# MPEGGroup/mpeg-pcc-tmc13

Hardware: AMD Instinct MI355X
Metric: RAHT forward+inverse attribute-transform Mpoints/s (bit-exact vs CPU reference) (higher is better)
Workload: dtype int64 (Q15 fixed point), int32 I/O

## Files before the change

### mpeg-pcc-tmc13_amd/csrc/cx_level.hpp

```cpp
#pragma once

#include "cx_tree.hpp"
#include "raht_arith.hpp"
#include "raht_levels.hpp"
#include "raht_links.hpp"
#include "raht_rdoq.hpp"

#ifndef GPCC_CX_SEARCH_ARY
#define GPCC_CX_SEARCH_ARY 2
#endif
#ifndef GPCC_CX_SEARCH_MASKED
#define GPCC_CX_SEARCH_MASKED 0
#endif

namespace gpcc {

constexpr int kCxG = 57;
constexpr int kCxSlices = 64;
constexpr int kCxTopTiles = 8;

struct CxCtx {
  TreeView tv;
  CxLists cl;
  const gpcc_raht_params* params;
// ... 128 lines not shown
{
  if (w <= 65536)
    return (int64_t)(1 + (((w << 30) * (rs40 >> 15)) >> 40));
  return (int64_t)isqrt(w << (2 * kFpFrac), L.rsqrt);
}

__device__ __forceinline__ CxNorm
cx_norm(int32_t w, const SharedLut& L)
{
  CxNorm r;
  if (w < kSmallN) {
    r.sq = L.norm_sq[w];
    r.rs = L.norm_rs[w];
    r.shift = 0;
    return r;
  }
  const uint64_t rs40 = irsqrt((uint64_t)w, L.rsqrt);
  r.shift = w > 1024 ? ilog2_u64((uint64_t)w - 1) >> 1 : 0;
  r.rs = (int64_t)(rs40 >> (40 - r.shift - kFpFrac));
  r.sq = cx_sqrt_from_rsqrt((uint64_t)w, rs40, L);
  return r;
}

template<class A>
__device__ __forceinline__ typename A::T
cx_scale(typename A::T v, const CxNorm& nm, typename A::Coef rs)
{
  return A::mulc(A::shr(v, nm.shift), rs);
}

template<class VT>
__device__ __forceinline__ VT
cx_bperm_v(int src_lane, VT v)
{
  return __builtin_bit_cast(VT, cx_bperm_i64(src_lane, __builtin_bit_cast(int64_t, v)));
}

__device__ __forceinline__ void
cx_coeffs(
  int32_t wl, int32_t wr, int64_t sql, int64_t sqr, const SharedLut& L, int64_t* a, int64_t* b,
  int64_t* sqw)
{
  const uint64_t w = (uint64_t)wl + (uint64_t)wr;
  if (wl < kSmallW && wr < kSmallW) {
    *a = L.bfly_a[wl * kSmallW + wr];
    *b = L.bfly_b[wl * kSmallW + wr];
    *sqw = L.norm_sq[w];
    return;
  }
  const uint64_t rs = irsqrt(w, L.rsqrt);
  *a = (int64_t)(((uint64_t)sql * rs) >> 40);
  *b = (int64_t)(((uint64_t)sqr * rs) >> 40);
  *sqw = cx_sqrt_from_rsqrt(w, rs, L);
}

__device__ __forceinline__ uint32_t
cx_rdoq_threshold(int64_t dist2, int64_t lambda, double inv_lambda, int rate_coeff, uint32_t limit)
{
  const uint64_t d = (uint64_t)dist2 << 26;
  const uint64_t lam = (uint64_t)lambda;
  const int rc = (rate_coeff + 128) >> 8;
  constexpr uint64_t kCap = 128;
  uint64_t q = kCap;
  if (d < lam * kCap) {
    q = (uint64_t)((double)d * inv_lambda);
    q -= q * lam > d;
    q += (q + 1) * lam <= d;
  }
  const int m = (int)q - rc + 1;
  if (m <= 1)
    return 0;
  if (m <= 2)
    return 1;
  if (m <= 3)
    return 2;
  if (m <= 5)
    return 3;
  if (m <= 7)
    return 5;
  if (m <= 9)
    return 7;
  if (m <= 11)
    return 9;
  int bb = (m - 12 + 1) >> 1;
  bb = bb < 1 ? 1 : bb;
  if (bb > 30)
    return kDescNever;
  const uint32_t tz = 10u + (1u << (bb - 1));
  return tz > limit ? kDescNever : tz;
}

__device__ __forceinline__ void
cx_fill_quant(ParamsConst prm, const LevelSched& e, int c, CxQuant* qt, int entry)
{
  int a0 = 0, a1 = 0;
  const int pos = entry - 1;
  if (pos >= 1 && e.ac_layer < prm->num_ac_qp_layers) {
    a0 = prm->ac_qp_offset[e.ac_layer][pos - 1][0];
    a1 = prm->ac_qp_offset[e.ac_layer][pos - 1][1];
  }
  Quantizer q[2];
  qpset_quantizers(prm, e.qp_layer, a0, a1, q);
  qt->q[entry][0] = q[0];
  qt->q[entry][1] = q[1];
  if (entry == 0) {
    const int64_t l0 = q[0].step;
    qt->lambda = l0 * l0 * (c == 1 ? 25 : 35);
    qt->inv_lambda = 1.0 / (double)qt->lambda;
  }
}

#ifdef GPCC_CX_PROF
__device__ unsigned long long g_cx_prof[16];
__device__ unsigned long long g_cx_prof_n[4];
struct CxProf {
  unsigned long long last;
  __device__ CxProf() { last = __builtin_amdgcn_s_memtime(); }
  __device__ void mark(int phase)
  {
    const unsigned long long t = __builtin_amdgcn_s_memtime();
    if (lane_id() == 0)
      atomicAdd(&g_cx_prof[phase], t - last);
    last = t;
  }
  __device__ void count(int slot, unsigned n)
  {
    if (lane_id() == 0)
      atomicAdd(&g_cx_prof[slot], (unsigned long long)n);
  }
};
#else
struct CxProf {
  __device__ void mark(int) {}
  __device__ void count(int, unsigned) {}
};
#endif

template<int C>
__device__ __forceinline__ void
cx_level_setup(const CxCtx& cx, CxSmem& sm, int li)
{
  const ParamsConst prm = (ParamsConst)cx.params;
// ... 427 lines not shown
  Quantizer qa[2], qr[2];
  int64_t lambda;
  double inv_lambda;
  if (S <= kCxSlices) {
    const CxQuant& qt = sm.qt[s];
    qa[0] = qt.q[1 + pos][0];
    qa[1] = qt.q[1 + pos][1];
    qr[0] = qt.q[0][0];
    qr[1] = qt.q[0][1];
    lambda = qt.lambda;
    inv_lambda = qt.inv_lambda;
  } else {
    int ac0 = 0, ac1 = 0;
    if (e.ac_layer < prm->num_ac_qp_layers && pos) {
      ac0 = prm->ac_qp_offset[e.ac_layer][pos - 1][0];
      ac1 = prm->ac_qp_offset[e.ac_layer][pos - 1][1];
    }
    qpset_quantizers(prm, e.qp_layer, ac0, ac1, qa);
    qpset_quantizers(prm, e.qp_layer, 0, 0, qr);
    const int64_t l0 = qr[0].step;
    lambda = l0 * l0 * (C == 1 ? 25 : 35);
    inv_lambda = 1.0 / (double)lambda;
  }

  const typename A::Quant qaa[2] = {A::quant(qa[0]), A::quant(qa[1])};
  int32_t qco[C];
#pragma unroll
  for (int k = 0; k < C; k++)
    qco[k] = 0;
  if (ENC) {
    uint32_t d = kDescZero;
    if (coded) {
      if (enable_pred) {
#pragma unroll
        for (int k = 0; k < C; k++)
          src[k] -= pred[k];
      }
      const typename A::Quant qra[2] = {A::quant(qr[0]), A::quant(qr[1])};
      int64_t sum_coeff = 0, dist2 = 0;
      int rate_coeff = 0;
#pragma unroll
      for (int k = 0; k < C; k++) {
        const VT co = A::round_int(src[k]);
        const int64_t coi = A::to_small(co);
        dist2 += coi * coi;
        int64_t aq = A::quantize(qra[k ? 1 : 0], co);
        aq = aq < 0 ? -aq : aq;
        sum_coeff += aq;
        rate_coeff += rate_log_small(aq);
        qco[k] = A::quantize(qaa[k ? 1 : 0], co);
      }
      d = kDescNever;
      if (sum_coeff < 3) {
        d = cx_rdoq_threshold(dist2, lambda, inv_lambda, rate_coeff, (uint32_t)sl.n_s);
        if (sum_coeff == 0)
          d |= kDescZero;
      }
    }

    prof.mark(4);
    const unsigned long long ep = (unsigned long long)(li + 1) << 48;
    unsigned long long todo = __ballot(coded);
    bool zero_me = false;
    bool published = false;
    while (todo) {
      const int first = __ffsll((long long)todo) - 1;
      const int s_cur = __shfl(s, first);
      const int c_first = __shfl(cblock, first);
      const bool mine = coded && s == s_cur;
      const unsigned long long seg = __ballot(mine);
      todo &= ~seg;
      const bool last_seg = todo == 0;
      const int ncoef = __popcll(seg);
      const int e_base = __shfl(e.coeff_base, first);
      const int e_par = __shfl((int)e.parity, first);
      const int c_end = __shfl(sl.coeff_end, first);
      if (mine)
        wdesc[cidx - c_first] = d;
      __builtin_amdgcn_wave_barrier();
      const bool valid = lane < ncoef;
      const uint32_t dd = valid ? wdesc[lane] : kDescZero;
      const int ci = c_first + lane;
      const bool starts = c_first == e_base;
      const bool ends = c_first + ncoef == c_end;
      int l_in = 0, l_out = 0;
      int tz;
      if (starts) {
        l_in = cx.slice_l[(e_par ^ 1) * S + s_cur];
        l_out = rdoq_chunk(dd, ci, valid, l_in, c_first, &tz);
        if (last_seg && lane == 0)
          __hip_atomic_store(
            &cx.tstate[tile], ep | (3ull << 32) | (uint32_t)l_out, __ATOMIC_RELAXED, __HIP_MEMORY_SCOPE_AGENT);
        published = published || last_seg;
      } else {
        const int la0 = -1, lb0 = c_first - 1;
        int tza, tzb;
        const int la = rdoq_chunk(dd, ci, valid, la0, c_first, &tza);
        const int lb = rdoq_chunk(dd, ci, valid, lb0, c_first, &tzb);
        const int status = lb == lb0 ? kTileTransparent : (la == lb ? kTileClosed : kTileOpen);
        if (last_seg && status != kTileOpen) {
          if (lane == 0)
            __hip_atomic_store(
              &cx.tstate[tile],
              ep | ((unsigned long long)(status == kTileClosed ? 2 : 1) << 32)
                | (uint32_t)(status == kTileClosed ? la : ncoef),
              __ATOMIC_RELAXED, __HIP_MEMORY_SCOPE_AGENT);
          published = true;
// ... 192 lines not shown
```

### mpeg-pcc-tmc13_amd/csrc/raht_levels.hpp

```cpp
#pragma once

#include "raht_common.hpp"

namespace gpcc {

enum LevelMode { kAnalyze = 0, kSynth = 1, kFused = 2, kLossySub = 3 };

constexpr uint32_t kDescNever = 0x7fffffffu;
constexpr uint32_t kDescZero = 0x80000000u;

typedef const __attribute__((address_space(4))) gpcc_raht_params* ParamsConst;

struct InterRef {
  const int64_t* pos;
  const int32_t* prefix;
  int32_t n_ref;
  int32_t lr;
  int32_t blocks;
  int32_t dual;
  int32_t filtered;
  const int32_t* tap;
  const int64_t* hkey;
  const int32_t* hfp;
  const int32_t* hlf;
// ... 155 lines not shown
  const int qp0 = clip(p->layer_qp[layer][0] + off0, 4, p->max_qp);
  const int qp1 = clip(p->layer_qp[layer][1] + off1 + qp0, 4, p->max_qp);
  q[0] = make_quantizer(qp0 + p->fixed_point_qp_offset);
  q[1] = make_quantizer(qp1 + p->fixed_point_qp_offset);
}

__device__ __forceinline__ int
find_in_window(
  const int64_t* __restrict__ key, int first, int last, int from,
  int64_t value, int64_t d)
{
  int lo, end;
  if (d >= 0) {
    lo = from;
    end = (d + 1 < (int64_t)(last - from)) ? from + (int)(d + 1) : last;
  } else {
    end = from;
    lo = (-d < (int64_t)(from - first)) ? from - (int)(-d) : first;
  }
  int hi = end;
  while (lo < hi) {
    const int mid = lo + ((hi - lo) >> 1);
    if (key[mid] < value)
      lo = mid + 1;
    else
      hi = mid;
  }
  if (lo == end)
    return -1;
  return key[lo] == value ? lo : -1;
}

__device__ __forceinline__ uint32_t
neigh_mask(int i)
{
  constexpr uint8_t m[19] = {255, 240, 204, 170, 192, 160, 136, 3,  5, 15,
                             17,  51,  85,  10,  34,  12,  68,  48, 80};
  return m[i];
}
__device__ __forceinline__ uint32_t
neigh_offset(int i)
{
  constexpr uint8_t o[19] = {0, 35, 21, 14, 49, 42, 28, 1,  2, 3,
                             4, 5,  6,  10, 12, 17, 20, 33, 34};
  return o[i];
}

__device__ __forceinline__ int
rate_log_small(int64_t aq)
{
  return aq == 0 ? 0 : (aq == 1 ? 256 : 406);
}

__device__ __forceinline__ uint32_t
rdoq_threshold(int64_t dist2, int64_t lambda, int rate_coeff, uint32_t limit)
{
  const uint64_t d = (uint64_t)dist2 << 26;
  const uint64_t lam = (uint64_t)lambda;
  const int rc = (rate_coeff + 128) >> 8;
  constexpr uint64_t kCap = 128;
  uint64_t q = kCap;
  if (d < lam * kCap) {
    q = (uint64_t)((double)d / (double)lam);
    q -= q * lam > d;
    q += (q + 1) * lam <= d;
  }
  const int m = (int)q - rc + 1;
  if (m <= 1)
    return 0;
  if (m <= 2)
    return 1;
  if (m <= 3)
    return 2;
  if (m <= 5)
    return 3;
  if (m <= 7)
    return 5;
  if (m <= 9)
    return 7;
  if (m <= 11)
    return 9;
  int bb = (m - 12 + 1) >> 1;
  bb = bb < 1 ? 1 : bb;
  if (bb > 30)
    return kDescNever;
  const uint32_t tz = 10u + (1u << (bb - 1));
  return tz > limit ? kDescNever : tz;
}

template<int C>
__global__ __launch_bounds__(256) void
raht_level_prepass_kernel(LevelCtx ctx)
{
  __shared__ int wave_cnt[4];
  __shared__ int base_s;
  if (tree_failed(ctx.tv))
    return;
  const TreeView& tv = ctx.tv;
  const int li = ctx.li;
  const bool ext = ctx.params->raht_extension != 0;
  const int num_parents = tv.soff[li + 1][tv.num_slices];
  const int lane = lane_id(), wave = threadIdx.x >> 6;
  if (ctx.rdoq_state && ctx.slice_l && blockIdx.x == 0)
    for (int s = threadIdx.x; s < tv.num_slices; s += blockDim.x)
      ctx.slice_l[(li & 1) * tv.num_slices + s] = ctx.slice_l[((li + 1) & 1) * tv.num_slices + s];
  const int64_t chunks = ((int64_t)num_parents + 255) >> 8;
  const int64_t per = (chunks + gridDim.x - 1) / gridDim.x;
  const int64_t gbeg = min((int64_t)blockIdx.x * per, chunks);
  const int64_t gend = min(gbeg + per, chunks);

  int mine = 0;
  for (int64_t chunk = gbeg; chunk < gend; chunk++) {
    const int j = (int)(chunk * 256) + threadIdx.x;
    if (j < num_parents) {
      const int s = find_slice(tv.soff[li + 1], tv.num_slices, j);
      if (ctx.sched[s].lvl[li].processed) {
        const int nchild = tv.fc[li + 1][j + 1] - tv.fc[li + 1][j];
        mine += !(ext && nchild == 1);
      }
    }
  }
#pragma unroll
  for (int d = 1; d < kWave; d <<= 1)
    mine += __shfl_xor(mine, d);
  if (lane == 0)
    wave_cnt[wave] = mine;
  __syncthreads();
  if (threadIdx.x == 0) {
    const unsigned long long ep = (unsigned long long)(li + 1) << 48;
    const unsigned total = wave_cnt[0] + wave_cnt[1] + wave_cnt[2] + wave_cnt[3];
    unsigned excl = 0;
    if (blockIdx.x > 0) {
      __hip_atomic_store(
        &ctx.scan_state[blockIdx.x], ep | (1ull << 32) | total, __ATOMIC_RELAXED,
        __HIP_MEMORY_SCOPE_AGENT);
      int k = (int)blockIdx.x - 1;
      for (;;) {
        const unsigned long long v = __hip_atomic_load(
          &ctx.scan_state[k], __ATOMIC_RELAXED, __HIP_MEMORY_SCOPE_AGENT);
        if ((v >> 48) != (unsigned long long)(li + 1)) {
// ... 70 lines not shown
```

### mpeg-pcc-tmc13_amd/csrc/raht_subnode.hpp

```cpp
#pragma once

#include <stdlib.h>

#include "raht_arith.hpp"
#include "raht_inter.hpp"
#include "raht_levels.hpp"
#include "raht_links.hpp"

namespace gpcc {

#ifndef GPCC_SUB_CHUNK
#define GPCC_SUB_CHUNK 1
#endif
#ifndef GPCC_SUB_DSTORE
#define GPCC_SUB_DSTORE 0
#endif
#ifndef GPCC_SUB_POLL_N
#define GPCC_SUB_POLL_N 1
#endif
#ifndef GPCC_SUB_IDLE_FAST
#define GPCC_SUB_IDLE_FAST 1
#endif
#ifndef GPCC_SUB_IDLE_SPIN
#define GPCC_SUB_IDLE_SPIN 0
#endif
__device__ __forceinline__ int64_t
sub_round_of_ticket(int tk, int cls)
{
  constexpr int K = GPCC_SUB_CHUNK;
  return ((int64_t)(tk / K) * 8 + cls) * K + tk % K;
}

#ifdef GPCC_SUB_PROF
__device__ unsigned long long g_sub_prof[16 + 32 * 20];
struct SubProf {
  unsigned long long t0 = 0, t1 = 0, last = 0, acc[4] = {0, 0, 0, 0}, iters = 0, idle_iters = 0;
  unsigned long long last2 = 0, sub_acc[6] = {0, 0, 0, 0, 0, 0}, execs[2] = {0, 0};
  template<int WHICH> __device__ void enter() { execs[WHICH]++; last2 = now(); }
  template<int K> __device__ void sub() { const unsigned long long t = now(); sub_acc[K] += t - last2; last2 = t; }
  __device__ static unsigned long long now() { return __builtin_amdgcn_s_memtime(); }
  __device__ void round_begin() { t0 = now(); }
  __device__ void loop_begin() { t1 = now(); }
  __device__ void iter_begin() { last = now(); iters++; }
  template<int STAGE> __device__ void mark() { const unsigned long long t = now(); acc[STAGE] += t - last; last = t; }
  __device__ void idle() { idle_iters++; }
  __device__ void round_end(int lane, int li)
  {
    if (lane != 0)
      return;
    const unsigned long long t2 = now();
    const unsigned long long v[9] = {1, t1 - t0, t2 - t1, acc[0], acc[1], acc[2], acc[3], iters, idle_iters};
    for (int i = 0; i < 9; i++)
      atomicAdd(&g_sub_prof[i], v[i]);
    atomicAdd(&g_sub_prof[16 + li * 4 + 0], 1ull);
    atomicAdd(&g_sub_prof[16 + li * 4 + 1], t1 - t0);
    atomicAdd(&g_sub_prof[16 + li * 4 + 2], t2 - t1);
    atomicAdd(&g_sub_prof[16 + li * 4 + 3], iters);
    for (int i = 0; i < 4; i++)
      atomicAdd(&g_sub_prof[144 + li * 6 + i], acc[i]);
    atomicAdd(&g_sub_prof[144 + li * 6 + 4], idle_iters);
    atomicAdd(&g_sub_prof[336 + li * 10 + 0], execs[0]);
    atomicAdd(&g_sub_prof[336 + li * 10 + 1], execs[1]);
    for (int i = 0; i < 6; i++)
      atomicAdd(&g_sub_prof[336 + li * 10 + 2 + i], sub_acc[i]);
  }
};
#else
struct SubProf {
  __device__ void round_begin() {}
  __device__ void loop_begin() {}
  __device__ void iter_begin() {}
  template<int STAGE> __device__ void mark() {}
  template<int WHICH> __device__ void enter() {}
  template<int K> __device__ void sub() {}
  __device__ void idle() {}
  __device__ void round_end(int, int) {}
};
// ... 4 lines not shown
{
#if GPCC_EXPERIMENTS
  auto rounds = [] {
    const char* e = getenv("GPCC_SUB_CLAIM");
    const int v = e ? atoi(e) : 1;
    return v < 1 ? 1 : (v > 64 ? 64 : v);
  };
  auto limit = [] {
    const char* e = getenv("GPCC_SUB_CLAIM_PARENTS");
    return e ? (int64_t)atoll(e) : (int64_t)100000;
  };
#ifdef GPCC_EMU
  const int r = rounds();
  const int64_t lim = limit();
#else
  static const int r = rounds();
  static const int64_t lim = limit();
#endif
  return (encoder && !haar && r > 1 && parents <= lim) ? r : 1;
#else
  (void)encoder;
  (void)haar;
  (void)parents;
  return 1;
#endif
}

__device__ __forceinline__ int
occu_shift(int i12)
{
  constexpr uint8_t s[12] = {6, 5, 4, 3, 2, 1, 3, 1, 2, 1, 2, 3};
  return s[i12];
}

__device__ __forceinline__ int32_t
load_agent_i32(const int32_t* p)
{
  return __hip_atomic_load(p, __ATOMIC_RELAXED, __HIP_MEMORY_SCOPE_AGENT);
}
__device__ __forceinline__ int64_t
load_agent_i64(const int64_t* p)
{
  return __hip_atomic_load(p, __ATOMIC_RELAXED, __HIP_MEMORY_SCOPE_AGENT);
}
__device__ __forceinline__ void
store_agent_i64(int64_t* p, int64_t v)
{
  __hip_atomic_store(p, v, __ATOMIC_RELAXED, __HIP_MEMORY_SCOPE_AGENT);
}

#ifndef GPCC_SUB_SLEEP
#define GPCC_SUB_SLEEP 4
#endif
#ifndef GPCC_SUB_POLL_RR
#define GPCC_SUB_POLL_RR 0
#endif
#ifndef GPCC_SUB_LOSSY_WAVES
#define GPCC_SUB_LOSSY_WAVES 3
#endif
#ifndef GPCC_SUB_SYNTH3_WAVES
#define GPCC_SUB_SYNTH3_WAVES 4
#endif
template<int C, int MODE, class A = ArithI64, bool INTER = false, bool REC = false>
__global__ __launch_bounds__(256, MODE == kLossySub ? GPCC_SUB_LOSSY_WAVES : (C == 3 ? GPCC_SUB_SYNTH3_WAVES : 4)) void
raht_level_sub_kernel(LevelCtx ctx)
{
  static_assert(!(REC && (INTER || MODE == kFused)), "records: fixed-point intra kernels only");
  static_assert(MODE == kSynth || MODE == kFused || MODE == kLossySub, "mode");
  static_assert(!(A::kF64 && MODE == kFused), "integer Haar is integer arithmetic");
  typedef typename A::T VT;
  typedef typename A::Coef VC;
  constexpr bool kLossy = MODE == kLossySub;
  __shared__ SharedLut lut_s;
  if (tree_failed(ctx.tv))
    return;
  load_lut(&lut_s, ctx.lut);
  const SharedLut& lut = lut_s;

  constexpr bool kEnc = MODE != kSynth;
  constexpr bool kRecon = true;
  const TreeView& tv = ctx.tv;
  const ParamsConst prm = (ParamsConst)ctx.params;
  const int li = ctx.li;
  const int t = threadIdx.x & 7;
  const int lane = lane_id();
  const int gbase = threadIdx.x & 56;
  const bool haar = !A::kF64 && prm->integer_haar_enable_flag != 0;
  const bool ext = A::kF64 || prm->raht_extension != 0;
  const int32_t epoch = li + 1;
#ifdef GPCC_EMU
  __shared__ unsigned long long wmail_s[8 * 4 * 64 * C];
  unsigned long long* wm = wmail_s + ((blockIdx.x & 7) * 4 + (threadIdx.x >> 6)) * (64 * C);
#else
  __shared__ unsigned long long wmail_s[4 * 64 * C];
  unsigned long long* wm = wmail_s + (threadIdx.x >> 6) * (64 * C);
#endif
  int pwc12[12];
#pragma unroll
  for (int i12 = 0; i12 < 12; i12++)
    pwc12[i12] = prm->pred_weight_child[i12];
  bool in_range = true;
  const int cls = blockIdx.x & 7;

  const int num_work = ctx.work_count[li];
#if GPCC_EXPERIMENTS
  const int claim_rounds = ctx.claim_rounds > 1 ? ctx.claim_rounds : 1;
  bool stop_all = false;
  for (;;) {
    int tk = 0;
    if (lane == 0)
      tk = atomicAdd(&ctx.ticket[li * 8 + (claim_rounds > 1 ? 0 : cls)], 1);
    tk = __shfl(tk, 0);
    const int64_t wround0 = claim_rounds > 1 ? (int64_t)tk * claim_rounds : sub_round_of_ticket(tk, cls);
    if (wround0 * 8 >= num_work || stop_all)
      break;
    bool carry_known = false;
    int carry_l = -1;
   for (int sr = 0; sr < claim_rounds; sr++) {
    const int64_t wround = wround0 + sr;
    if (wround * 8 >= num_work)
      break;
    SubProf prof;
    prof.round_begin();
    if (__hip_atomic_load(ctx.error, __ATOMIC_RELAXED, __HIP_MEMORY_SCOPE_AGENT)) {
      stop_all = true;
      break;
    }
#else
  for (;;) {
    int tk = 0;
    if (lane == 0)
      tk = atomicAdd(&ctx.ticket[li * 8 + cls], 1);
    tk = __shfl(tk, 0);
    const int64_t wround = sub_round_of_ticket(tk, cls);
    if (wround * 8 >= num_work)
      break;
    SubProf prof;
    prof.round_begin();
    if (__hip_atomic_load(ctx.error, __ATOMIC_RELAXED, __HIP_MEMORY_SCOPE_AGENT))
      break;
#endif
    const int wi = (int)(wround * 8) + (lane >> 3);
    const bool live = wi < num_work;
    const int j = live ? ctx.worklist[wi] : 0;
    int s = 0;
    LevelSched e;
    e.processed = 0;
    const size_t rln = REC ? (size_t)ctx.brec.lanes : 0;
    const size_t rat = (size_t)wround * 64 + lane;
    const int32_t* __restrict__ rf = REC ? ctx.brec.f32 + rat : nullptr;
    if (live) {
      if constexpr (REC)
        s = rf[kSfSlice * rln];
// ... 313 lines not shown
    const VC nrm_sq = A::coef(nrm_sq_i), nrm_rs = A::coef(nrm_rs_i);
    const typename A::Quant qaa[2] = {A::quant(qa[0]), A::quant(qa[1])};
    if (kEnc && !REC) {
      if (!haar && w > 1) {
#pragma unroll
        for (int k = 0; k < C; k++)
          src[k] = A::mulc(A::shr(src[k], nrm_shift), nrm_rs);
      }
#pragma unroll
      for (int k = 0; k < C; k++)
        in_range = in_range && A::below(src[k], A::kFwdLimit);
#pragma unroll
      for (int st = 0; st < 3; st++) {
        const int bit = 1 << st;
        const bool left = !(t & bit);
        const bool both = wl[st] && wr[st];
        const bool swap = !wl[st] && wr[st];
#pragma unroll
        for (int k = 0; k < C; k++) {
          const VT own = src[k], oth = shfl_xor_v(own, bit);
          if (both) {
            if (haar) {
              if constexpr (!A::kF64) {
                const int64_t hf = left ? oth - own : own - oth;
                src[k] = left ? own + ((hf >> (1 + kFpFrac)) << kFpFrac) : hf;
              }
            } else {
              src[k] = left ? A::mulc(oth, cb[st]) + A::mulc(own, ca[st])
                            : A::mulc(own, ca[st]) - A::mulc(oth, cb[st]);
            }
          } else if (swap) {
            src[k] = oth;
          }
        }
      }
    }
    const uint32_t coded_mask = group8_bits(coded);
    const int ncoef = popc32(coded_mask);
    const int crank = inherit_dc ? rank - 1 : rank;
    const int cfirst = e.coeff_base + (inherit_dc ? (c0 - sc0) - pj : 0);
    int rank_src = 0;
    if (kLossy) {
#pragma unroll
      for (int u = 0; u < 8; u++) {
        const int ru = __shfl(crank, gbase | u);
        if (((coded_mask >> u) & 1) && ru == t)
          rank_src = u;
      }
    }
    Quantizer qr[2] = {{1, 1}, {1, 1}};
    if (kLossy && coded)
      qpset_quantizers(prm, e.qp_layer, nq0, nq1, qr);
    const typename A::Quant qra[2] = {A::quant(qr[0]), A::quant(qr[1])};
    bool lin_known = false;
    int lin = -1;
    VT dc[C];
#pragma unroll
    for (int k = 0; k < C; k++)
      dc[k] = A::zero();
    if (on && inherit_dc && t == 0) {
#pragma unroll
      for (int k = 0; k < C; k++) {
        const int64_t val = par2(ctx.rec_us, par_par)[prow * C + k];
        dc[k] = A::from_i64(
          ext ? val : (val > 0 ? val << (kFpFrac - 2) : -((-val) << (kFpFrac - 2))));
        in_range = in_range && A::below(dc[k], A::kInvLimit);
      }
    }

    const bool run = do_search && enable_pred;
    const int64_t* __restrict__ prec = par2(ctx.rec, par_par);
    const int64_t rbase = (int64_t)pt0 - sp0;
    int wsum = 0;
    VT lim_lo = A::zero(), lim_hi = A::zero();
#pragma unroll
    for (int i = 0; i < 7; i++) {
      int q;
      if (i == 0)
        q = j;
      else
        q = __shfl(pn[0], gbase | (i - 1));
      if (!run || q < 0)
        continue;
      VT v[C];
#pragma unroll
      for (int k = 0; k < C; k++) {
        v[k] = A::from_i64(prec[(rbase + q) * C + k]);
        in_range = in_range && A::below(v[k], A::kRecLimit);
      }
      if (i) {
        if (A::muli(v[0], 10) <= lim_lo || A::muli(v[0], 10) >= lim_hi)
          continue;
      } else {
        lim_lo = A::muli(v[0], 2);
        lim_hi = A::muli(v[0], 25);
      }
      if (has && ((neigh_mask(i) >> t) & 1)) {
        const int pw = prm->pred_weight_parent[i];
        wsum += pw;
        const int mul = ext ? pw : (pw << kFpFrac);
#pragma unroll
        for (int k = 0; k < C; k++)
          pred[k] += A::muli(v[k], mul);
      }
    }

    int nb_c0[3] = {0, 0, 0};
    uint32_t nb_occ[3] = {0, 0, 0};
    int nb_single[3] = {0, 0, 0};
    VT nb_v[3][C];
#pragma unroll
    for (int slot = 0; slot < 3; slot++) {
#pragma unroll
      for (int k = 0; k < C; k++)
        nb_v[slot][k] = A::zero();
      const int i = 1 + t + 8 * slot;
      if (run && i >= 7 && i < 19 && pn[slot] >= 0) {
        const int q = pn[slot];
#pragma unroll
        for (int k = 0; k < C; k++) {
          nb_v[slot][k] = A::from_i64(prec[(rbase + q) * C + k]);
          in_range = in_range && A::below(nb_v[slot][k], A::kRecLimit);
        }
        if constexpr (REC) {
          nb_c0[slot] = rf[(kSfNbc0 + slot) * rln];
          nb_occ[slot] = (rpk >> (8 * slot)) & 0xffu;
          nb_single[slot] = (int)((rpk >> (24 + slot)) & 1u);
        } else if (q < j) {
          const int qc0 = tv.fc[li + 1][q];
          nb_c0[slot] = qc0;
          nb_occ[slot] = ctx.pocc[q];
          nb_single[slot] = ext && tv.fc[li + 1][q + 1] - qc0 == 1;
        }
      }
    }
    uint32_t pend = 0;
    int32_t nrow12[12];
    uint32_t inw = 0, wsrc_a = 0, wsrc_b = 0;
    int jg[8];
#pragma unroll
    for (int g = 0; g < 8; g++)
      jg[g] = __shfl(on ? j : -1, g << 3);
#pragma unroll
    for (int i12 = 0; i12 < 12; i12++) {
      nrow12[i12] = 0;
      const int i = 7 + i12;
      const int owner = gbase | ((i - 1) & 7);
      const int sl = (i - 1) >> 3;
      const int q = __shfl(pn[sl], owner);
      const int qc0 = __shfl(nb_c0[sl], owner);
      const uint32_t qocc = __shfl(nb_occ[sl], owner);
      const int single = __shfl(nb_single[sl], owner);
      VT v[C];
#pragma unroll
      for (int k = 0; k < C; k++)
        v[k] = shfl_v(nb_v[sl][k], owner);
      if (!run || q < 0)
        continue;
      if (A::muli(v[0], 10) <= lim_lo || A::muli(v[0], 10) >= lim_hi)
        continue;
      if (has && ((neigh_mask(i) >> t) & 1)) {
        const int sh = occu_shift(i12);
        const int cpos = i12 < 9 ? t + sh : t - sh;
        const bool child_ok = cpos >= 0 && cpos < 8 && ((qocc >> cpos) & 1);
        if (child_ok) {
          const int cidx_n = qc0 + popc32(qocc & ((1u << cpos) - 1));
          const int64_t nrow = (int64_t)pt0 + (cidx_n - sc0);
          const int pwc = prm->pred_weight_child[i12];
          wsum += pwc;
          if (single) {
            const int mul = ext ? pwc : (pwc << kFpFrac);
#pragma unroll
            for (int k = 0; k < C; k++) {
              const VT cv = A::from_i64(par2(ctx.rec, cur_par)[nrow * C + k]);
              in_range = in_range && A::below(cv, A::kRecLimit);
              pred[k] += A::muli(cv, mul);
            }
          } else {
            nrow12[i12] = (int32_t)nrow;
            pend |= 1u << i12;
            int pg = -1;
#pragma unroll
            for (int g = 0; g < 7; g++)
              pg = q == jg[g] ? g : pg;
            if (pg >= 0) {
              inw |= 1u << i12;
              if (i12 < 10)
                wsrc_a |= (uint32_t)pg << (3 * i12);
              else
                wsrc_b |= (uint32_t)pg << (3 * (i12 - 10));
            }
          }
        } else {
          const int pwp = prm->pred_weight_parent[i];
          wsum += pwp;
          const int mul = ext ? pwp : (pwp << kFpFrac);
#pragma unroll
          for (int k = 0; k < C; k++)
            pred[k] += A::muli(v[k], mul);
        }
      }
    }
    const VC pdiv = A::coef(pred_divisor(wsum > 0 ? wsum : 1));
    const auto mrsrc = __builtin_amdgcn_make_buffer_rsrc(
      ctx.mbox, 0, (int)((size_t)tv.n_total * C * 16), 0x00020000);

    bool use_inter = false;
    VT ipin[C];
#pragma unroll
    for (int k = 0; k < C; k++)
      ipin[k] = A::zero();
    if constexpr (INTER) {
      if (ctx.inter.blocks) {
        bool node;
        int64_t pin[C];
        if (ctx.inter.hkey)
          inter_block_haar<C>(ctx.inter, on ? tv.key[li + 1][j] : 0, t, on, &node, pin);
        else
          inter_block<C>(ctx.inter, on ? tv.key[li + 1][j] : 0, t, on, lut, &node, pin);
        use_inter = node;
#pragma unroll
        for (int k = 0; k < C; k++) {
          ipin[k] = A::from_i64(pin[k]);
          in_range = in_range && (!node || A::below(ipin[k], A::kFwdLimit));
        }
        if (use_inter) {
          pend = 0;
          inw = 0;
          enable_pred = on;
        }
      }
    }

    int stage = on ? 0 : 3;
    unsigned spins = 0;
    VT pt[C];
    int32_t qc[C];
    uint32_t dr = kDescZero;
    int zs = 0;
    bool zero_r = false;
    uint32_t dmask = 0;
    bool lin_exact = false;
    int need = 0;
    int look = wi - 1;
    int outk = 0, outv = -1;
    unsigned long long done = 0;
    int poll_last = 31;
    unsigned long long done_seen = ~0ull;
    int cur_slot = -1, cur_pwc = 0;
    int32_t cur_row = 0;
    int cur_mul = 0;
#pragma unroll
    for (int k = 0; k < C; k++) {
      pt[k] = A::zero();
      qc[k] = (!kEnc && coded) ? cplane[(size_t)k * n_s] : 0;
    }
    prof.loop_begin();
    while (__any(stage != 3)) {
      bool progressed = false;
      prof.iter_begin();
      if (!GPCC_SUB_IDLE_FAST || done != done_seen) {
        done_seen = done;
        uint32_t mi = stage == 0 ? (pend & inw) : 0u;
        while (__any(mi != 0)) {
          const bool act = mi != 0;
          const int slot = act ? __ffs(mi) - 1 : 0;
          mi &= mi - 1;
          const uint32_t pg = (slot < 10 ? wsrc_a >> (3 * slot) : wsrc_b >> (3 * (slot - 10))) & 7u;
          constexpr unsigned long long kShifts = 06ull | 05ull << 3 | 04ull << 6 | 03ull << 9 | 02ull << 12
            | 01ull << 15 | 03ull << 18 | 01ull << 21 | 02ull << 24 | 01ull << 27 | 02ull << 30 | 03ull << 33;
          const int sh = (int)((kShifts >> (3 * slot)) & 7);
          const int srcl = (int)(pg << 3) | ((slot < 9 ? t + sh : t - sh) & 7);
          if (act && ((done >> srcl) & 1)) {
            int pwc = 0;
#pragma unroll
            for (int i12 = 0; i12 < 12; i12++)
              pwc = slot == i12 ? pwc12[i12] : pwc;
            const int mul = ext ? pwc : (pwc << kFpFrac);
#pragma unroll
            for (int k = 0; k < C; k++)
              pred[k] += A::muli(__builtin_bit_cast(VT, wm[srcl * C + k]), mul);
            pend &= ~(1u << slot);
            inw &= ~(1u << slot);
          }
        }
      }
      const uint32_t pm = stage == 0 ? (pend & ~inw) : 0u;
#if GPCC_SUB_POLL_N > 1
      if (pm) {
        uint32_t pmm = pm;
        int slot_[GPCC_SUB_POLL_N], pwc_[GPCC_SUB_POLL_N];
        bool act_[GPCC_SUB_POLL_N];
        u32x4 g[GPCC_SUB_POLL_N][C];
#pragma unroll
        for (int u = 0; u < GPCC_SUB_POLL_N; u++) {
          act_[u] = pmm != 0;
          slot_[u] = act_[u] ? __ffs(pmm) - 1 : __ffs(pm) - 1;
          pmm &= pmm - 1;
          int32_t row = 0;
          pwc_[u] = 0;
#pragma unroll
          for (int i12 = 0; i12 < 12; i12++) {
            if (slot_[u] == i12) {
              row = nrow12[i12];
              pwc_[u] = pwc12[i12];
            }
          }
#pragma unroll
          for (int k = 0; k < C; k++)
            g[u][k] = __builtin_amdgcn_raw_buffer_load_b128(mrsrc, (row * C + k) * 16, 0,  16);
        }
#pragma unroll
        for (int u = 0; u < GPCC_SUB_POLL_N; u++) {
          bool ok = act_[u];
#pragma unroll
          for (int k = 0; k < C; k++)
            ok = ok && g[u][k].z == ctx.mtag;
          if (ok) {
            const int mul = ext ? pwc_[u] : (pwc_[u] << kFpFrac);
#pragma unroll
            for (int k = 0; k < C; k++)
              pred[k] += A::muli(__builtin_bit_cast(VT, ((uint64_t)g[u][k].y << 32) | g[u][k].x), mul);
            pend &= ~(1u << slot_[u]);
          }
        }
      }
#else
      if (pm) {
#if GPCC_SUB_POLL_RR
        const uint32_t above = pm & ~((2u << poll_last) - 1u);
        const int slot = __ffs(above ? above : pm) - 1;
        poll_last = slot;
#else
        const int slot = __ffs(pm) - 1;
#endif
        int32_t row = 0;
        int pwc = 0;
        if (GPCC_SUB_IDLE_FAST && !GPCC_SUB_POLL_RR) {
          if (slot != cur_slot) {
            cur_slot = slot;
#pragma unroll
            for (int i12 = 0; i12 < 12; i12++) {
              if (slot == i12) {
                cur_row = nrow12[i12];
                cur_pwc = pwc12[i12];
              }
            }
          }
          row = cur_row;
          pwc = cur_pwc;
        } else {
#pragma unroll
          for (int i12 = 0; i12 < 12; i12++) {
            if (slot == i12) {
              row = nrow12[i12];
              pwc = prm->pred_weight_child[i12];
            }
          }
        }
#if GPCC_SUB_IDLE_SPIN
        cur_mul = ext ? pwc : (pwc << kFpFrac);
      }
      {
        const bool spin_ok = !__any(stage == 1) && !__any(stage == 0 && !group8_any(stage == 0 && pend));
        u32x4 g[C];
        bool ok = false;
        bool expired = false;
        for (;;) {
          if (pm) {
#pragma unroll
            for (int k = 0; k < C; k++)
              g[k] = __builtin_amdgcn_raw_buffer_load_b128(mrsrc, (cur_row * C + k) * 16, 0,  16);
            ok = true;
#pragma unroll
            for (int k = 0; k < C; k++)
              ok = ok && g[k].z == ctx.mtag;
          }
          if (!spin_ok || __any(ok) || !__any(pm != 0))
            break;
          prof.idle();
          if (++spins > (1u << 21)) {
            expired = true;
            break;
          }
          __builtin_amdgcn_s_sleep(GPCC_SUB_SLEEP);
        }
        if (expired) {
          if (lane == 0)
            atomicExch(ctx.error, 1);
          break;
        }
        if (ok) {
#pragma unroll
          for (int k = 0; k < C; k++)
            pred[k] += A::muli(__builtin_bit_cast(VT, ((uint64_t)g[k].y << 32) | g[k].x), cur_mul);
          pend &= ~(1u << cur_slot);
        }
      }
#else
        u32x4 g[C];
#pragma unroll
        for (int k = 0; k < C; k++)
          g[k] = __builtin_amdgcn_raw_buffer_load_b128(mrsrc, (row * C + k) * 16, 0,  16);
        bool ok = true;
#pragma unroll
        for (int k = 0; k < C; k++)
          ok = ok && g[k].z == ctx.mtag;
        if (ok) {
          const int mul = ext ? pwc : (pwc << kFpFrac);
#pragma unroll
          for (int k = 0; k < C; k++)
            pred[k] += A::muli(__builtin_bit_cast(VT, ((uint64_t)g[k].y << 32) | g[k].x), mul);
          pend &= ~(1u << slot);
        }
      }
#endif
#endif
      prof.mark<0>();
      const bool blocked = group8_any(stage == 0 && pend);
      const bool nready = stage == 0 && !blocked;

      if (__any(nready)) {
        progressed = true;
        prof.template enter<0>();
        VT pw_[C];
#pragma unroll
        for (int k = 0; k < C; k++)
          pw_[k] = pred[k];
        if (run && has) {
#pragma unroll
          for (int k = 0; k < C; k++) {
            pw_[k] = A::mulc(pw_[k], pdiv);
            if constexpr (!A::kF64) {
              if (haar)
                pw_[k] = (pw_[k] >> kFpFrac) << kFpFrac;
            }
          }
        }
        if (!haar && w > 1 && enable_pred) {
#pragma unroll
          for (int k = 0; k < C; k++)
            pw_[k] = A::mulc(pw_[k], nrm_sq);
        }
#pragma unroll
        for (int k = 0; k < C; k++)
          in_range = in_range && A::below(pw_[k], A::kFwdLimit);
#pragma unroll
        for (int st = 0; st < 3; st++) {
          const int bit = 1 << st;
          const bool left = !(t & bit);
          const bool both = wl[st] && wr[st];
          const bool swap = !wl[st] && wr[st];
#pragma unroll
          for (int k = 0; k < C; k++) {
            const VT own = pw_[k], oth = shfl_xor_v(own, bit);
            if (enable_pred) {
              if (both) {
                if (haar) {
                  if constexpr (!A::kF64) {
                    const int64_t hf = left ? oth - own : own - oth;
                    pw_[k] = left ? own + ((hf >> (1 + kFpFrac)) << kFpFrac) : hf;
                  }
                } else {
                  pw_[k] = left ? A::mulc(oth, cb[st]) + A::mulc(own, ca[st])
                                : A::mulc(own, ca[st]) - A::mulc(oth, cb[st]);
                }
              } else if (swap) {
                pw_[k] = oth;
              }
            }
          }
        }
        if constexpr (INTER) {
          if (use_inter) {
#pragma unroll
            for (int k = 0; k < C; k++)
              pw_[k] = ipin[k];
          }
        }
        prof.template sub<0>();
        uint32_t d = kDescZero;
        int32_t qn_[C];
#pragma unroll
        for (int k = 0; k < C; k++)
          qn_[k] = 0;
        if (kEnc && coded) {
          int64_t sum_coeff = 0, dist2 = 0;
          int rate_coeff = 0;
#pragma unroll
          for (int k = 0; k < C; k++) {
            const VT res = enable_pred ? src[k] - pw_[k] : src[k];
            const VT co = A::round_int(res);
            qn_[k] = A::quantize(qaa[k ? 1 : 0], co);
            if (kLossy) {
              const int64_t coi = A::to_small(co);
              dist2 += coi * coi;
              int64_t aq = q_same ? (int64_t)qn_[k] : (int64_t)A::quantize(qra[k ? 1 : 0], co);
              aq = aq < 0 ? -aq : aq;
              sum_coeff += aq;
              rate_coeff += rate_log_small(aq);
            }
          }
          if (kLossy) {
            d = kDescNever;
            if (sum_coeff < 3) {
              bool any = false;
#pragma unroll
              for (int k = 0; k < C; k++)
                any |= qn_[k] != 0;
              if (sum_coeff == 0 && !any) {
                d = kDescZero;
              } else {
                const int64_t l0 = qr[0].step;
                d = rdoq_threshold(dist2, l0 * l0 * (C == 1 ? 25 : 35), rate_coeff, (uint32_t)n_s);
                if (sum_coeff == 0)
                  d |= kDescZero;
              }
            }
          }
        }
        prof.template sub<1>();
        uint32_t drn = kDescZero;
        if (kLossy) {
          const uint32_t du = __shfl(d, gbase | rank_src);
          drn = t < ncoef ? du : kDescZero;
        }
        if (nready) {
#pragma unroll
          for (int k = 0; k < C; k++) {
            pt[k] = pw_[k];
            if (kEnc)
              qc[k] = qn_[k];
          }
          dr = drn;
          stage = 1;
        }
      }

      prof.mark<1>();
      bool can = stage == 1;
      if (kLossy) {
        const bool rvalid = t < ncoef;
        const bool rz = dr >> 31;
        const uint32_t rthr = dr & kDescNever;
        const bool isthr = rvalid && !rz && rthr != kDescNever && rthr != 0;
        const bool dep = rvalid && rthr != kDescNever && rthr != 0;
        const int ci = cfirst + t;
        const uint32_t below = (1u << t) - 1u;
        auto resets_for = [&](int l0, bool act) -> uint32_t {
          uint32_t resets = dmask;
          for (;;) {
            const uint32_t bb = resets & below;
            const int lhat = bb ? cfirst + (31 - __clz(bb)) : l0;
            const bool fail = act && isthr && !((resets >> t) & 1) && (uint32_t)(ci - lhat) <= rthr;
            const unsigned long long m = __ballot(fail);
            if (!m)
              break;
            resets |= (uint32_t)(m >> gbase) & 0xffu;
          }
          return resets;
        };
        auto zeroed = [&](uint32_t resets, int l0) -> bool {
          const uint32_t bb = resets & below;
          const int lhat = bb ? cfirst + (31 - __clz(bb)) : l0;
          return rvalid && rthr != kDescNever && (uint32_t)(ci - 1 - lhat) >= rthr;
        };
        const bool entry = stage == 1 && zs == 0;
// ... 74 lines not shown
              } else if (fkind == 5) {
                lin = fval - 1;
                lin_known = true;
              } else {
                look -= first;
              }
            }
          }
          const unsigned long long lead = 0x0101010101010101ull;
          const unsigned long long before = (1ull << gbase) - 1;
          for (int pass = 0; pass < 8; pass++) {
            const bool settle = stage == 1 && zs == 1 && lin_known;
            if (__any(settle)) {
              const uint32_t rr = resets_for(lin, settle);
              if (settle) {
                zero_r = zeroed(rr, lin);
                zs = 2;
                if (rr) {
                  outk = 2;
                  outv = cfirst + (31 - __clz(rr));
                } else if (lin_exact) {
                  outk = 2;
                  outv = lin;
                } else {
                  outk = 1;
                }
              }
            }
            const bool w2 = stage == 1 && zs == 1 && !lin_known;
            if (!__any(w2))
              break;
            const unsigned long long nt = __ballot(outk != 1) & lead & before;
            const int pl = nt ? 63 - __clzll((long long)nt) : 0;
            const int pk = __shfl(outk, pl);
            const int pv = __shfl(outv, pl);
#if GPCC_EXPERIMENTS
            const bool from_carry = w2 && nt == 0 && carry_known;
            const bool found = (w2 && nt != 0 && pk == 2) || from_carry;
            if (found) {
              lin = from_carry ? carry_l : pv;
              lin_known = lin_exact = true;
            }
#else
            const bool found = w2 && nt != 0 && pk == 2;
            if (found) {
              lin = pv;
              lin_known = lin_exact = true;
            }
#endif
            if (!__any(found))
              break;
          }
        }
        can = stage == 1 && zs == 2;
        if (can && t == 0) {
          const unsigned long long ep = (unsigned long long)epoch << 48;
          const unsigned long long word =
            outk >= 2 ? ep | (2ull << 32) | (uint32_t)outv : ep | (1ull << 32) | (uint32_t)cfirst;
          __hip_atomic_store(&ctx.rdoq_state[wi], word, __ATOMIC_RELAXED, __HIP_MEMORY_SCOPE_AGENT);
          if (outk >= 2)
            atomicMax(&ctx.slice_l[(li & 1) * tv.num_slices + s], outv);
        }
      }

      prof.mark<2>();
      if (__any(can)) {
        progressed = true;
        prof.template enter<1>();
        VT pw_[C];
#pragma unroll
        for (int k = 0; k < C; k++)
          pw_[k] = pt[k];
        bool zero_me = false;
        if (kLossy)
          zero_me = __shfl((int)zero_r, gbase | (crank & 7)) != 0 && coded;
        if (coded && can) {
#pragma unroll
          for (int k = 0; k < C; k++) {
            int32_t co;
            if (kEnc) {
              co = zero_me ? 0 : qc[k];
              cplane[(size_t)k * n_s] = co;
            } else {
              co = qc[k];
            }
            pw_[k] += A::dequant_fp(qaa[k ? 1 : 0], co);
          }
        }
        if (on && inherit_dc && t == 0) {
#pragma unroll
          for (int k = 0; k < C; k++)
            pw_[k] = dc[k];
        }
#pragma unroll
        for (int k = 0; k < C; k++)
          in_range = in_range && A::below(pw_[k], A::kInvLimit);
#pragma unroll
        for (int st = 2; st >= 0; st--) {
          const int bit = 1 << st;
          const bool left = !(t & bit);
          const bool both = wl[st] && wr[st];
          const bool swap = !wl[st] && wr[st];
#pragma unroll
          for (int k = 0; k < C; k++) {
            const VT own = pw_[k], oth = shfl_xor_v(own, bit);
            if (both) {
              if (haar) {
                if constexpr (!A::kF64) {
                  const int64_t lf = left ? own : oth, hf = left ? oth : own;
                  const int64_t lv = lf - ((hf >> (1 + kFpFrac)) << kFpFrac);
                  pw_[k] = left ? lv : hf + lv;
                }
              } else {
                pw_[k] = left ? A::mulc(own, ca[st]) - A::mulc(oth, cb[st])
                              : A::mulc(oth, cb[st]) + A::mulc(own, ca[st]);
              }
            } else if (swap) {
              pw_[k] = oth;
            }
          }
        }
        prof.template sub<2>();
        if (can && has) {
          VT vn[C];
#pragma unroll
          for (int k = 0; k < C; k++) {
            VT v = pw_[k];
            if (!haar && w > 1)
              v = A::mulc(A::shr(v, nrm_shift), nrm_rs);
            v = ext ? v : A::round_int(v);
            vn[k] = v;
            const uint64_t vb = __builtin_bit_cast(uint64_t, v);
            wm[lane * C + k] = vb;
            const u32x4 gr = {(uint32_t)vb, (uint32_t)(vb >> 32), ctx.mtag, 0u};
#if GPCC_SUB_DSTORE
            __builtin_amdgcn_raw_buffer_store_b128(gr, mrsrc, (int)((crow * C + k) * 16), 0, 0);
#endif
            __builtin_amdgcn_raw_buffer_store_b128(gr, mrsrc, (int)((crow * C + k) * 16), 0,  16);
          }
          prof.template sub<3>();
#pragma unroll
          for (int k = 0; k < C; k++) {
            par2(ctx.rec_us, cur_par)[crow * C + k] = A::to_i64(ext ? pw_[k] : A::round_int(A::muli(pw_[k], 4)));
            par2(ctx.rec, cur_par)[crow * C + k] = A::to_i64(vn[k]);
          }
          par2(ctx.nneigh, cur_par)[crow] = inherit_dc ? neigh_count : 19;
          prof.template sub<4>();
        }
        if (can)
          stage = 3;
      }

      done |= __ballot(can && has);
      prof.mark<3>();
      if (!progressed) {
        prof.idle();
        if (++spins > (1u << 21)) {
          if (lane == 0)
            atomicExch(ctx.error, 1);
          break;
        }
        __builtin_amdgcn_s_sleep(GPCC_SUB_SLEEP);
      }
    }
    prof.round_end(lane, li);
#if GPCC_EXPERIMENTS
    if (kLossy && claim_rounds > 1) {
      const unsigned long long fin = __ballot(outk == 2) & 0x0101010101010101ull;
      if (fin) {
        carry_l = __shfl(outv, 63 - __clzll((long long)fin));
        carry_known = true;
      } else if (__any(outk == 1)) {
        carry_known = false;
      }
    }
   }
#endif
  }
  if (A::kF64 && __any(!in_range) && lane == 0)
    atomicCAS(ctx.error, 0, 3);
}

}
```

Baseline: 91.13.

## Overlap mailbox polling loads with butterfly work in subnode kernel

The subnode kernel now issues the neighbour mailbox loads early and consumes them later, after the butterfly and RDOQ work has run, so global-memory latency is hidden behind compute. Per-slot neighbour rows and prediction weights move from register arrays into LDS, which cuts register pressure and drops the 12-way select loops. The RDOQ threshold now uses a reciprocal lambda computed once per node instead of a division, and the F64 butterfly is made branchless. Several experimental polling knobs are removed. The risks are extra LDS use and explicit waitcnt and asm barriers that may stall if they are placed wrongly.

```diff
diff --git a/mpeg-pcc-tmc13_amd/csrc/cx_level.hpp b/mpeg-pcc-tmc13_amd/csrc/cx_level.hpp
--- a/mpeg-pcc-tmc13_amd/csrc/cx_level.hpp
+++ b/mpeg-pcc-tmc13_amd/csrc/cx_level.hpp
@@ -204,42 +204,6 @@
   *a = (int64_t)(((uint64_t)sql * rs) >> 40);
   *b = (int64_t)(((uint64_t)sqr * rs) >> 40);
   *sqw = cx_sqrt_from_rsqrt(w, rs, L);
-}
-
-__device__ __forceinline__ uint32_t
-cx_rdoq_threshold(int64_t dist2, int64_t lambda, double inv_lambda, int rate_coeff, uint32_t limit)
-{
-  const uint64_t d = (uint64_t)dist2 << 26;
-  const uint64_t lam = (uint64_t)lambda;
-  const int rc = (rate_coeff + 128) >> 8;
-  constexpr uint64_t kCap = 128;
-  uint64_t q = kCap;
-  if (d < lam * kCap) {
-    q = (uint64_t)((double)d * inv_lambda);
-    q -= q * lam > d;
-    q += (q + 1) * lam <= d;
-  }
-  const int m = (int)q - rc + 1;
-  if (m <= 1)
-    return 0;
-  if (m <= 2)
-    return 1;
-  if (m <= 3)
-    return 2;
-  if (m <= 5)
-    return 3;
-  if (m <= 7)
-    return 5;
-  if (m <= 9)
-    return 7;
-  if (m <= 11)
-    return 9;
-  int bb = (m - 12 + 1) >> 1;
-  bb = bb < 1 ? 1 : bb;
-  if (bb > 30)
-    return kDescNever;
-  const uint32_t tz = 10u + (1u << (bb - 1));
-  return tz > limit ? kDescNever : tz;
 }
 
 __device__ __forceinline__ void
@@ -773,7 +737,7 @@
       }
       d = kDescNever;
       if (sum_coeff < 3) {
-        d = cx_rdoq_threshold(dist2, lambda, inv_lambda, rate_coeff, (uint32_t)sl.n_s);
+        d = rdoq_threshold_recip(dist2, lambda, inv_lambda, rate_coeff, (uint32_t)sl.n_s);
         if (sum_coeff == 0)
           d |= kDescZero;
       }
diff --git a/mpeg-pcc-tmc13_amd/csrc/raht_levels.hpp b/mpeg-pcc-tmc13_amd/csrc/raht_levels.hpp
--- a/mpeg-pcc-tmc13_amd/csrc/raht_levels.hpp
+++ b/mpeg-pcc-tmc13_amd/csrc/raht_levels.hpp
@@ -231,19 +231,12 @@
   return aq == 0 ? 0 : (aq == 1 ? 256 : 406);
 }
 
+constexpr uint64_t kRdoqCap = 128;
+
 __device__ __forceinline__ uint32_t
-rdoq_threshold(int64_t dist2, int64_t lambda, int rate_coeff, uint32_t limit)
-{
-  const uint64_t d = (uint64_t)dist2 << 26;
-  const uint64_t lam = (uint64_t)lambda;
+rdoq_threshold_of_quotient(uint64_t q, int rate_coeff, uint32_t limit)
+{
   const int rc = (rate_coeff + 128) >> 8;
-  constexpr uint64_t kCap = 128;
-  uint64_t q = kCap;
-  if (d < lam * kCap) {
-    q = (uint64_t)((double)d / (double)lam);
-    q -= q * lam > d;
-    q += (q + 1) * lam <= d;
-  }
   const int m = (int)q - rc + 1;
   if (m <= 1)
     return 0;
@@ -265,6 +258,34 @@
     return kDescNever;
   const uint32_t tz = 10u + (1u << (bb - 1));
   return tz > limit ? kDescNever : tz;
+}
+
+__device__ __forceinline__ uint32_t
+rdoq_threshold(int64_t dist2, int64_t lambda, int rate_coeff, uint32_t limit)
+{
+  const uint64_t d = (uint64_t)dist2 << 26;
+  const uint64_t lam = (uint64_t)lambda;
+  uint64_t q = kRdoqCap;
+  if (d < lam * kRdoqCap) {
+    q = (uint64_t)((double)d / (double)lam);
+    q -= q * lam > d;
+    q += (q + 1) * lam <= d;
+  }
+  return rdoq_threshold_of_quotient(q, rate_coeff, limit);
+}
+
+__device__ __forceinline__ uint32_t
+rdoq_threshold_recip(int64_t dist2, int64_t lambda, double inv_lambda, int rate_coeff, uint32_t limit)
+{
+  const uint64_t d = (uint64_t)dist2 << 26;
+  const uint64_t lam = (uint64_t)lambda;
+  uint64_t q = kRdoqCap;
+  if (d < lam * kRdoqCap) {
+    q = (uint64_t)((double)d * inv_lambda);
+    q -= q * lam > d;
+    q += (q + 1) * lam <= d;
+  }
+  return rdoq_threshold_of_quotient(q, rate_coeff, limit);
 }
 
 template<int C>
diff --git a/mpeg-pcc-tmc13_amd/csrc/raht_subnode.hpp b/mpeg-pcc-tmc13_amd/csrc/raht_subnode.hpp
--- a/mpeg-pcc-tmc13_amd/csrc/raht_subnode.hpp
+++ b/mpeg-pcc-tmc13_amd/csrc/raht_subnode.hpp
@@ -14,15 +14,6 @@
 #endif
 #ifndef GPCC_SUB_DSTORE
 #define GPCC_SUB_DSTORE 0
-#endif
-#ifndef GPCC_SUB_POLL_N
-#define GPCC_SUB_POLL_N 1
-#endif
-#ifndef GPCC_SUB_IDLE_FAST
-#define GPCC_SUB_IDLE_FAST 1
-#endif
-#ifndef GPCC_SUB_IDLE_SPIN
-#define GPCC_SUB_IDLE_SPIN 0
 #endif
 __device__ __forceinline__ int64_t
 sub_round_of_ticket(int tk, int cls)
@@ -133,9 +124,6 @@
 #ifndef GPCC_SUB_SLEEP
 #define GPCC_SUB_SLEEP 4
 #endif
-#ifndef GPCC_SUB_POLL_RR
-#define GPCC_SUB_POLL_RR 0
-#endif
 #ifndef GPCC_SUB_LOSSY_WAVES
 #define GPCC_SUB_LOSSY_WAVES 3
 #endif
@@ -176,10 +164,19 @@
   __shared__ unsigned long long wmail_s[4 * 64 * C];
   unsigned long long* wm = wmail_s + (threadIdx.x >> 6) * (64 * C);
 #endif
-  int pwc12[12];
-#pragma unroll
-  for (int i12 = 0; i12 < 12; i12++)
-    pwc12[i12] = prm->pred_weight_child[i12];
+#ifdef GPCC_EMU
+  __shared__ int32_t nrow_s[8][12][256];
+  __shared__ int32_t pwc_s[8 * 4][12];
+#define GPCC_SUB_NROW(i12) nrow_s[blockIdx.x & 7][i12][threadIdx.x]
+#define GPCC_SUB_PWC(i12) pwc_s[(blockIdx.x & 7) * 4 + (threadIdx.x >> 6)][i12]
+#else
+  __shared__ int32_t nrow_s[12][256];
+  __shared__ int32_t pwc_s[4][12];
+#define GPCC_SUB_NROW(i12) nrow_s[i12][threadIdx.x]
+#define GPCC_SUB_PWC(i12) pwc_s[threadIdx.x >> 6][i12]
+#endif
+  if (lane < 12)
+    GPCC_SUB_PWC(lane) = prm->pred_weight_child[lane];
   bool in_range = true;
   const int cls = blockIdx.x & 7;
 
@@ -599,6 +596,8 @@
     if (kLossy && coded)
       qpset_quantizers(prm, e.qp_layer, nq0, nq1, qr);
     const typename A::Quant qra[2] = {A::quant(qr[0]), A::quant(qr[1])};
+    const int64_t rd_lambda = (int64_t)qr[0].step * qr[0].step * (C == 1 ? 25 : 35);
+    const double rd_inv_lambda = 1.0 / (double)rd_lambda;
     bool lin_known = false;
     int lin = -1;
     VT dc[C];
@@ -682,7 +681,6 @@
       }
     }
     uint32_t pend = 0;
-    int32_t nrow12[12];
     uint32_t inw = 0, wsrc_a = 0, wsrc_b = 0;
     int jg[8];
 #pragma unroll
@@ -690,7 +688,6 @@
       jg[g] = __shfl(on ? j : -1, g << 3);
 #pragma unroll
     for (int i12 = 0; i12 < 12; i12++) {
-      nrow12[i12] = 0;
       const int i = 7 + i12;
       const int owner = gbase | ((i - 1) & 7);
       const int sl = (i - 1) >> 3;
@@ -724,7 +721,7 @@
               pred[k] += A::muli(cv, mul);
             }
           } else {
-            nrow12[i12] = (int32_t)nrow;
+            GPCC_SUB_NROW(i12) = (int32_t)nrow;
             pend |= 1u << i12;
             int pg = -1;
 #pragma unroll
@@ -792,21 +789,22 @@
     int look = wi - 1;
     int outk = 0, outv = -1;
     unsigned long long done = 0;
-    int poll_last = 31;
     unsigned long long done_seen = ~0ull;
     int cur_slot = -1, cur_pwc = 0;
     int32_t cur_row = 0;
-    int cur_mul = 0;
 #pragma unroll
     for (int k = 0; k < C; k++) {
       pt[k] = A::zero();
       qc[k] = (!kEnc && coded) ? cplane[(size_t)k * n_s] : 0;
     }
+#ifndef GPCC_EMU
+    __builtin_amdgcn_s_waitcnt(0x0f70);
+#endif
     prof.loop_begin();
     while (__any(stage != 3)) {
       bool progressed = false;
       prof.iter_begin();
-      if (!GPCC_SUB_IDLE_FAST || done != done_seen) {
+      if (done != done_seen) {
         done_seen = done;
         uint32_t mi = stage == 0 ? (pend & inw) : 0u;
         while (__any(mi != 0)) {
@@ -819,10 +817,7 @@
           const int sh = (int)((kShifts >> (3 * slot)) & 7);
           const int srcl = (int)(pg << 3) | ((slot < 9 ? t + sh : t - sh) & 7);
           if (act && ((done >> srcl) & 1)) {
-            int pwc = 0;
-#pragma unroll
-            for (int i12 = 0; i12 < 12; i12++)
-              pwc = slot == i12 ? pwc12[i12] : pwc;
+            const int pwc = GPCC_SUB_PWC(slot);
             const int mul = ext ? pwc : (pwc << kFpFrac);
 #pragma unroll
             for (int k = 0; k < C; k++)
@@ -833,138 +828,52 @@
         }
       }
       const uint32_t pm = stage == 0 ? (pend & ~inw) : 0u;
-#if GPCC_SUB_POLL_N > 1
+      u32x4 g[C];
       if (pm) {
-        uint32_t pmm = pm;
-        int slot_[GPCC_SUB_POLL_N], pwc_[GPCC_SUB_POLL_N];
-        bool act_[GPCC_SUB_POLL_N];
-        u32x4 g[GPCC_SUB_POLL_N][C];
-#pragma unroll
-        for (int u = 0; u < GPCC_SUB_POLL_N; u++) {
-          act_[u] = pmm != 0;
-          slot_[u] = act_[u] ? __ffs(pmm) - 1 : __ffs(pm) - 1;
-          pmm &= pmm - 1;
-          int32_t row = 0;
-          pwc_[u] = 0;
-#pragma unroll
-          for (int i12 = 0; i12 < 12; i12++) {
-            if (slot_[u] == i12) {
-              row = nrow12[i12];
-              pwc_[u] = pwc12[i12];
-            }
-          }
-#pragma unroll
-          for (int k = 0; k < C; k++)
-            g[u][k] = __builtin_amdgcn_raw_buffer_load_b128(mrsrc, (row * C + k) * 16, 0,  16);
-        }
-#pragma unroll
-        for (int u = 0; u < GPCC_SUB_POLL_N; u++) {
-          bool ok = act_[u];
-#pragma unroll
-          for (int k = 0; k < C; k++)
-            ok = ok && g[u][k].z == ctx.mtag;
+        const int slot = __ffs(pm) - 1;
+        if (slot != cur_slot) {
+          cur_slot = slot;
+          cur_row = GPCC_SUB_NROW(slot);
+          cur_pwc = GPCC_SUB_PWC(slot);
+        }
+#pragma unroll
+        for (int k = 0; k < C; k++)
+          g[k] = __builtin_amdgcn_raw_buffer_load_b128(mrsrc, (cur_row * C + k) * 16, 0,  16);
+      }
+      auto take_poll = [&]() -> bool {
+        bool ok = pm != 0;
+        if (pm) {
+#pragma unroll
+          for (int k = 0; k < C; k++) {
+#ifndef GPCC_EMU
+            asm volatile("" : : "v"(g[k]));
+#endif
+            ok = ok && g[k].z == ctx.mtag;
+          }
           if (ok) {
-            const int mul = ext ? pwc_[u] : (pwc_[u] << kFpFrac);
+            const int mul = ext ? cur_pwc : (cur_pwc << kFpFrac);
 #pragma unroll
             for (int k = 0; k < C; k++)
-              pred[k] += A::muli(__builtin_bit_cast(VT, ((uint64_t)g[u][k].y << 32) | g[u][k].x), mul);
-            pend &= ~(1u << slot_[u]);
-          }
-        }
-      }
-#else
-      if (pm) {
-#if GPCC_SUB_POLL_RR
-        const uint32_t above = pm & ~((2u << poll_last) - 1u);
-        const int slot = __ffs(above ? above : pm) - 1;
-        poll_last = slot;
-#else
-        const int slot = __ffs(pm) - 1;
-#endif
-        int32_t row = 0;
-        int pwc = 0;
-        if (GPCC_SUB_IDLE_FAST && !GPCC_SUB_POLL_RR) {
-          if (slot != cur_slot) {
-            cur_slot = slot;
-#pragma unroll
-            for (int i12 = 0; i12 < 12; i12++) {
-              if (slot == i12) {
-                cur_row = nrow12[i12];
-                cur_pwc = pwc12[i12];
-              }
-            }
-          }
-          row = cur_row;
-          pwc = cur_pwc;
-        } else {
-#pragma unroll
-          for (int i12 = 0; i12 < 12; i12++) {
-            if (slot == i12) {
-              row = nrow12[i12];
-              pwc = prm->pred_weight_child[i12];
-            }
-          }
-        }
-#if GPCC_SUB_IDLE_SPIN
-        cur_mul = ext ? pwc : (pwc << kFpFrac);
-      }
-      {
-        const bool spin_ok = !__any(stage == 1) && !__any(stage == 0 && !group8_any(stage == 0 && pend));
-        u32x4 g[C];
-        bool ok = false;
-        bool expired = false;
-        for (;;) {
-          if (pm) {
-#pragma unroll
-            for (int k = 0; k < C; k++)
-              g[k] = __builtin_amdgcn_raw_buffer_load_b128(mrsrc, (cur_row * C + k) * 16, 0,  16);
-            ok = true;
-#pragma unroll
-            for (int k = 0; k < C; k++)
-              ok = ok && g[k].z == ctx.mtag;
-          }
-          if (!spin_ok || __any(ok) || !__any(pm != 0))
-            break;
-          prof.idle();
-          if (++spins > (1u << 21)) {
-            expired = true;
-            break;
-          }
-          __builtin_amdgcn_s_sleep(GPCC_SUB_SLEEP);
-        }
-        if (expired) {
-          if (lane == 0)
-            atomicExch(ctx.error, 1);
-          break;
-        }
-        if (ok) {
-#pragma unroll
-          for (int k = 0; k < C; k++)
-            pred[k] += A::muli(__builtin_bit_cast(VT, ((uint64_t)g[k].y << 32) | g[k].x), cur_mul);
-          pend &= ~(1u << cur_slot);
-        }
-      }
-#else
-        u32x4 g[C];
-#pragma unroll
-        for (int k = 0; k < C; k++)
-          g[k] = __builtin_amdgcn_raw_buffer_load_b128(mrsrc, (row * C + k) * 16, 0,  16);
-        bool ok = true;
-#pragma unroll
-        for (int k = 0; k < C; k++)
-          ok = ok && g[k].z == ctx.mtag;
-        if (ok) {
-          const int mul = ext ? pwc : (pwc << kFpFrac);
-#pragma unroll
-          for (int k = 0; k < C; k++)
-            pred[k] += A::muli(__builtin_bit_cast(VT, ((uint64_t)g[k].y << 32) | g[k].x), mul);
-          pend &= ~(1u << slot);
-        }
-      }
-#endif
-#endif
+              pred[k] += A::muli(__builtin_bit_cast(VT, ((uint64_t)g[k].y << 32) | g[k].x), mul);
+            pend &= ~(1u << cur_slot);
+          }
+        }
+        return ok;
+      };
+      bool blocked = group8_any(stage == 0 && pend);
+      bool poll_open = __any(stage == 0 && !blocked);
+      if (!poll_open) {
+        if (__any(take_poll()))
+          blocked = group8_any(stage == 0 && pend);
+      }
+      auto take_poll_behind = [&]() {
+#ifndef GPCC_EMU
+        __builtin_amdgcn_s_waitcnt(0x0f70);
+#endif
+        if (poll_open)
+          take_poll();
+      };
       prof.mark<0>();
-      const bool blocked = group8_any(stage == 0 && pend);
       const bool nready = stage == 0 && !blocked;
 
       if (__any(nready)) {
@@ -1001,7 +910,10 @@
 #pragma unroll
           for (int k = 0; k < C; k++) {
             const VT own = pw_[k], oth = shfl_xor_v(own, bit);
-            if (enable_pred) {
+            if constexpr (A::kF64) {
+              const VT bf = A::mulc(own, ca[st]) + A::mulc(left ? oth : -oth, cb[st]);
+              pw_[k] = !enable_pred ? own : (both ? bf : (swap ? oth : own));
+            } else if (enable_pred) {
               if (both) {
                 if (haar) {
                   if constexpr (!A::kF64) {
@@ -1058,8 +970,7 @@
               if (sum_coeff == 0 && !any) {
                 d = kDescZero;
               } else {
-                const int64_t l0 = qr[0].step;
-                d = rdoq_threshold(dist2, l0 * l0 * (C == 1 ? 25 : 35), rate_coeff, (uint32_t)n_s);
+                d = rdoq_threshold_recip(dist2, rd_lambda, rd_inv_lambda, rate_coeff, (uint32_t)n_s);
                 if (sum_coeff == 0)
                   d |= kDescZero;
               }
@@ -1240,6 +1151,7 @@
               break;
           }
         }
+        take_poll_behind();
         can = stage == 1 && zs == 2;
         if (can && t == 0) {
           const unsigned long long ep = (unsigned long long)epoch << 48;
@@ -1252,13 +1164,13 @@
       }
 
       prof.mark<2>();
+      VT pw_[C];
+#pragma unroll
+      for (int k = 0; k < C; k++)
+        pw_[k] = pt[k];
       if (__any(can)) {
         progressed = true;
         prof.template enter<1>();
-        VT pw_[C];
-#pragma unroll
-        for (int k = 0; k < C; k++)
-          pw_[k] = pt[k];
         bool zero_me = false;
         if (kLossy)
           zero_me = __shfl((int)zero_r, gbase | (crank & 7)) != 0 && coded;
@@ -1292,7 +1204,10 @@
 #pragma unroll
           for (int k = 0; k < C; k++) {
             const VT own = pw_[k], oth = shfl_xor_v(own, bit);
-            if (both) {
+            if constexpr (A::kF64) {
+              const VT bf = A::mulc(own, ca[st]) + A::mulc(left ? -oth : oth, cb[st]);
+              pw_[k] = both ? bf : (swap ? oth : own);
+            } else if (both) {
               if (haar) {
                 if constexpr (!A::kF64) {
                   const int64_t lf = left ? own : oth, hf = left ? oth : own;
@@ -1309,6 +1224,10 @@
           }
         }
         prof.template sub<2>();
+      }
+      if (!kLossy)
+        take_poll_behind();
+      if (__any(can)) {
         if (can && has) {
           VT vn[C];
 #pragma unroll
@@ -1367,6 +1286,8 @@
   }
   if (A::kF64 && __any(!in_range) && lane == 0)
     atomicCAS(ctx.error, 0, 3);
+#undef GPCC_SUB_NROW
+#undef GPCC_SUB_PWC
 }
 
 }
```

New measurement: 101.4 (median of 6 runs). 11.2% higher.
